# lmcinnes/pynndescent

Measured on AMD Instinct MI355X. Metric: index build: points indexed/sec (recall@10 vs brute force reported alongside), higher is better.
Workload: dtype f32

## Files before the change

### include/pynnd_amd.h

```cpp
#ifndef PYNND_AMD_H
#define PYNND_AMD_H

#include <stdint.h>

#ifdef __cplusplus
extern "C" {
#endif

#define NND_METRIC_SQEUCLIDEAN 0
#define NND_METRIC_ALT_COSINE 1
#define NND_METRIC_ALT_DOT 2
#define NND_METRIC_ALT_INNER_PRODUCT 3
#define NND_METRIC_CORRELATION 4
#define NND_METRIC_ALT_HELLINGER 5
enum { NND_METRIC_PROXY_INNER_PRODUCT = 6 };
enum {
    NND_METRIC_JACCARD = 8,
    NND_METRIC_DICE = 9,
    NND_METRIC_SOKALSNEATH = 10,
    NND_METRIC_MATCHING = 11,
    NND_METRIC_ROGERSTANIMOTO = 12,
    NND_METRIC_SOKALMICHENER = 13,
    NND_METRIC_KULSINSKI = 14,
    NND_METRIC_RUSSELLRAO = 15,
// ... 12 lines not shown
    int32_t n_trees;
    int32_t leaf_size;
    int32_t max_depth;
    int32_t max_candidates;
    int32_t n_iters;
    float delta;
    int64_t rng_state[3];
    int64_t tree_rng[3];
    int32_t device;
    int32_t join_blocks;
    int32_t flags;
    int32_t reserved[5];
} nnd_params;

#define NND_FLAG_NO_GRAPH 1
#define NND_FLAG_NO_PREP 2
#define NND_FLAG_TEST_SELECT_WAVE 4
#define NND_FLAG_TEST_SMALL_REGIONS 8
#define NND_FLAG_TEST_ROUTE_PLAIN 16
#define NND_FLAG_TEST_FOREST_BY_TREE 32
#define NND_FLAG_TEST_FAIL 64
#define NND_FLAG_TEST_VANISH 128
#define NND_FLAG_TEST_SAMPLE_ATOMIC 256
#define NND_FLAG_TEST_FOREST_FALLBACK_TOPS 512
#define NND_FLAG_TEST_FOREST_FALLBACK_SHARE 1024
#define NND_TEST_FALLBACK_AT(flags) ((((flags) & 512) ? 1 : 0) + (((flags) & 1024) ? 2 : 0))
#define NND_FLAG_TEST_SAMPLE_NOMEM 2048
#define NND_FLAG_TEST_SELECT_HALF 4096
#define NND_FLAG_TEST_GATHER_INLINE 8192
#define NND_FLAG_TEST_JOIN_UNSTAGED 16384

#define NND_FLAG_TEST_EXACT_F64 32768
#define NND_FLAG_TEST_RANDOM_INIT_ROWWISE 65536

typedef struct nnd_stats {
    int64_t n_iters_run;
    int64_t n_leaves;
    int64_t tree_levels;
    int64_t leaf_pairs;
    int64_t leaf_rows;
    int64_t join_pairs[64];
    int64_t join_rows[64];
    int64_t join_active[64];
    int64_t proposals[64];
    int64_t updates[64];
    float ms_prep, ms_forest, ms_leaf_init, ms_random_init, ms_descent, ms_finalize;
    float ms_sample[64], ms_join[64], ms_merge[64];
    int64_t join_mfma[64];
    int64_t leaf_mfma;
    int64_t n_cells;
    int64_t join_substeps[64];
} nnd_stats;

int32_t nnd_abi_version(void);
const char *nnd_last_global_error(void);
const char *nnd_last_error(nnd_handle_t h);

int32_t nnd_create(nnd_handle_t *out, const nnd_params *params);
int32_t nnd_destroy(nnd_handle_t h);
int32_t nnd_release_pending(void);

int32_t nnd_host_copy(void *dst, const void *src, int64_t bytes);
int32_t nnd_host_sqrt_f32(float *dst, const float *src, int64_t count);
void *nnd_host_alloc(int64_t bytes);
int32_t nnd_host_free(void *p);

// ... 254 lines not shown
```

### pynndescent_amd/_capi.py

```python
import ctypes as C
import os

import numpy as np

_HERE = os.path.dirname(os.path.abspath(__file__))
LIB_PATH = os.environ.get("PYNND_AMD_LIB", os.path.join(_HERE, "libpynnd_amd.so"))

NND_METRIC_SQEUCLIDEAN = 0
NND_METRIC_ALT_COSINE = 1
NND_METRIC_ALT_DOT = 2
NND_METRIC_ALT_INNER_PRODUCT = 3
NND_METRIC_CORRELATION = 4
NND_METRIC_ALT_HELLINGER = 5
NND_METRIC_PROXY_INNER_PRODUCT = 6
METRIC_CODES = {"euclidean": NND_METRIC_SQEUCLIDEAN, "l2": NND_METRIC_SQEUCLIDEAN, "sqeuclidean": NND_METRIC_SQEUCLIDEAN,
                "cosine": NND_METRIC_ALT_COSINE, "dot": NND_METRIC_ALT_DOT, "inner_product": NND_METRIC_ALT_INNER_PRODUCT,
                "correlation": NND_METRIC_CORRELATION, "hellinger": NND_METRIC_ALT_HELLINGER,
                "proxy_inner_product": NND_METRIC_PROXY_INNER_PRODUCT}
(NND_METRIC_JACCARD, NND_METRIC_DICE, NND_METRIC_SOKALSNEATH, NND_METRIC_MATCHING, NND_METRIC_ROGERSTANIMOTO,
 NND_METRIC_SOKALMICHENER, NND_METRIC_KULSINSKI, NND_METRIC_RUSSELLRAO, NND_METRIC_YULE) = range(8, 17)
BOOLEAN_METRIC_CODES = {"jaccard": NND_METRIC_JACCARD, "dice": NND_METRIC_DICE, "sokalsneath": NND_METRIC_SOKALSNEATH,
                        "matching": NND_METRIC_MATCHING, "rogerstanimoto": NND_METRIC_ROGERSTANIMOTO,
                        "sokalmichener": NND_METRIC_SOKALMICHENER, "kulsinski": NND_METRIC_KULSINSKI,
                        "russellrao": NND_METRIC_RUSSELLRAO, "yule": NND_METRIC_YULE}


def metric_code(name):
    return METRIC_CODES[name] if name in METRIC_CODES else BOOLEAN_METRIC_CODES[name]
NND_DTYPE_FLOAT32, NND_DTYPE_FLOAT16, NND_DTYPE_BFLOAT16, NND_DTYPE_FLOAT64 = 0, 1, 2, 3
NND_FILTER_MASK, NND_FILTER_IDS = 0, 1
NND_QUERY_FORMS = {"float": 0, "proxy": 1, "rerank": 2}
NND_CORRECT_COPY, NND_CORRECT_SQRT, NND_CORRECT_ALT_COSINE, NND_CORRECT_ALT_INNER_PRODUCT, NND_CORRECT_ALT_HELLINGER = 0, 1, 2, 3, 4
NND_LINEAR_DIAGONAL, NND_LINEAR_DENSE = 0, 1
NND_FLAG_NO_GRAPH = 1
NND_FLAG_NO_PREP = 2
NND_FLAG_TEST_SELECT_WAVE = 4
NND_FLAG_TEST_SMALL_REGIONS = 8
NND_FLAG_TEST_ROUTE_PLAIN = 16
NND_FLAG_TEST_FOREST_BY_TREE = 32
NND_FLAG_TEST_FAIL = 64
NND_FLAG_TEST_VANISH = 128
NND_FLAG_TEST_FOREST_FALLBACK_TOPS = 512
NND_FLAG_TEST_FOREST_FALLBACK_SHARE = 1024
NND_FLAG_TEST_GATHER_INLINE = 8192
NND_FLAG_TEST_JOIN_UNSTAGED = 16384
NND_FLAG_TEST_SELECT_HALF = 4096
NND_FLAG_TEST_SAMPLE_NOMEM = 2048
NND_FLAG_TEST_EXACT_F64 = 32768
NND_FLAG_TEST_RANDOM_INIT_ROWWISE = 65536
NND_FLAG_TEST_SAMPLE_ATOMIC = 256


class NNDParams(C.Structure):
    _fields_ = [
        ("n", C.c_int64),
        ("dim", C.c_int32),
        ("metric", C.c_int32),
        ("n_neighbors", C.c_int32),
        ("n_trees", C.c_int32),
        ("leaf_size", C.c_int32),
        ("max_depth", C.c_int32),
        ("max_candidates", C.c_int32),
        ("n_iters", C.c_int32),
        ("delta", C.c_float),
        ("rng_state", C.c_int64 * 3),
        ("tree_rng", C.c_int64 * 3),
        ("device", C.c_int32),
        ("join_blocks", C.c_int32),
        ("flags", C.c_int32),
        ("reserved", C.c_int32 * 5),
    ]


class NNDSearchGraphStats(C.Structure):
    _fields_ = [("forward_nnz", C.c_int64), ("reverse_nnz", C.c_int64), ("union_nnz", C.c_int64), ("final_nnz", C.c_int64),
                ("min_distance", C.c_float), ("max_degree_out", C.c_int32), ("ms_device", C.c_float), ("reserved", C.c_int32 * 3)]


class NNDStats(C.Structure):
    _fields_ = [
        ("n_iters_run", C.c_int64),
        ("n_leaves", C.c_int64),
# ... 972 lines not shown
```

### pynndescent_amd/csrc/rpforest.hip

```cpp
#include <atomic>
#include <chrono>

#include "common.h"
#include "metric.h"
#include "state.h"

#define RP_EPS 1e-8f

static constexpr int SCAN_ITEMS = 8;
static constexpr int SCAN_BLOCK = 256;
static constexpr int SCAN_TILE = SCAN_ITEMS * SCAN_BLOCK;

__global__ void k_forest_init(int32_t *__restrict__ perm, int32_t *__restrict__ pos_seg, uint8_t *__restrict__ leaf_flag,
                              int32_t *__restrict__ inv, int64_t n, int64_t P, int splittable) {
    int64_t g = (int64_t)blockIdx.x * blockDim.x + threadIdx.x;
    if (g >= P) return;
    int64_t t = g / n;
    int64_t i = g - t * n;
    perm[g] = (int32_t)i;
    inv[g] = splittable ? (int32_t)t : -1;
    pos_seg[g] = splittable ? (int32_t)t : -1;
    leaf_flag[g] = (!splittable && i == 0) ? 1 : 0;
}
__global__ void k_forest_init_segs(int32_t *__restrict__ seg_start, int32_t *__restrict__ seg_len, int n_trees,
// ... 482 lines not shown
        return;
    }
    int a = seg_start[s];
    int nl = nleft[s];
    int right;
    int64_t dest;
    if (nl < 0) {
        nl = -nl - 1;
        int off = (int)(g - a);
        right = off & 1;
        dest = right ? (int64_t)a + nl + (off >> 1) : (int64_t)a + (off >> 1);
    } else {
        int L = scan[g] - scan[a];
        right = side[g];
        dest = right ? (int64_t)a + nl + ((int)(g - a) - L) : (int64_t)a + L;
    }
    int32_t p = perm[g];
    perm_out[dest] = p;
    pos_seg_out[dest] = seg_child[2 * s + right];
    if (inv) inv[(g / n) * n + p] = seg_child[2 * s + right];
}

#ifndef NND_FIN_MAX
#define NND_FIN_MAX 2048
#endif
static constexpr int FIN_MAX = NND_FIN_MAX;
#ifndef NND_BIG_MAX
#define NND_BIG_MAX 8192
#endif
static constexpr int BIG_MAX = NND_BIG_MAX;
static constexpr int FIN_STACK = 40;
static constexpr int FIN_SMALL = 512;
static constexpr int FIN_WS = 40;

__device__ __forceinline__ void rp_top2_push(uint64_t &a, uint64_t &b, uint64_t k) {
    if (k < a) {
        b = a;
        a = k;
    } else if (k < b) {
        b = k;
    }
}
__device__ __forceinline__ uint64_t rp_shfl_xor_u64(uint64_t v, int o) {
    const uint32_t lo = (uint32_t)__shfl_xor((int)(uint32_t)v, o, 64), hi = (uint32_t)__shfl_xor((int)(uint32_t)(v >> 32), o, 64);
    return ((uint64_t)hi << 32) | lo;
}

struct rp_record {
    float *hf;
    uint16_t *hh;
    int32_t *child;
    int32_t *leaf_depth;
    int hs, node_top, down_base, lvl_end;
    int *counter, *overflow;
    int min_len, max_len;
};
struct rp_tree_map {
    int tree_bias = 0;
    const int32_t *tree_begin = nullptr;
    int n_tree_begin = 0;
};
__device__ __forceinline__ uint32_t rp_tree_of(const rp_tree_map &tm, int64_t a, int64_t n) {
    if (!tm.tree_begin) return (uint32_t)(a / n) + (uint32_t)tm.tree_bias;
    int t = 0;
    for (int q = 1; q < tm.n_tree_begin; q++) t = a >= tm.tree_begin[q] ? q : t;
    return (uint32_t)t;
}

template <bool BIG, int NTHR, int CAP, bool RECORD = false>
__global__ __launch_bounds__(NTHR, NTHR == 64 ? 5 : 1) void k_finish_subtrees(const float *__restrict__ xp, const uint16_t *__restrict__ xh,
                                                         const float2 *__restrict__ nr, int metric, int dp, int64_t n,
                                                         int32_t *__restrict__ perm,
                                                         const int32_t *__restrict__ seg_start,
                                                         const int32_t *__restrict__ seg_len,
                                                         const int32_t *__restrict__ seg_depth, int depth0, int n_segs,
                                                         int angular, uint32_t seed, int max_depth, int leaf_size,
                                                         uint8_t *__restrict__ leaf_flag, int32_t *__restrict__ tmp_g,
                                                         uint8_t *__restrict__ side_g, int fin_max,
                                                         int32_t *__restrict__ fin_start, int32_t *__restrict__ fin_len,
                                                         int32_t *__restrict__ fin_depth, long long *__restrict__ fin_count,
                                                         rp_tree_map tm, const float *__restrict__ scal, rp_record rec = rp_record{}) {
    extern __shared__ __attribute__((aligned(16))) unsigned char fsm[];
    const int s = blockIdx.x;
    if (s >= n_segs) return;
    const int a = seg_start[s], len = seg_len[s];
    if (len <= 0) return;
    if (RECORD && (len < rec.min_len || len > rec.max_len)) return;
    constexpr int NLDS = BIG ? 0 : CAP;
    constexpr int NW = NTHR / 64;
    int32_t *ids = BIG ? perm + a : (int32_t *)fsm;
    int32_t *tmp = BIG ? tmp_g + a : (int32_t *)fsm + NLDS;
    uint8_t *sd = BIG ? side_g + a : (uint8_t *)((int32_t *)fsm + 2 * NLDS);
    float *h = (float *)(fsm + (size_t)NLDS * 9);
    uint16_t *hb = (uint16_t *)(h + dp + 4);
    int32_t *stk = (int32_t *)(hb + dp);
    int32_t *wsum = stk + FIN_STACK * 4;
    uint64_t *wkeys = (uint64_t *)(wsum + 8);
    const int tid = threadIdx.x, lane = nnd_lane(), w = tid >> 6;
    const uint32_t seedt = seed ^ (rp_tree_of(tm, a, n) * 0x9E3779B9u);
    const float hsc = scal[0], hinv = 1.0f / hsc, inv_s2 = scal[1];
    float cellA = 0.0f, cellB = 0.0f;
    if (!BIG) {
        for (int i = tid; i < len; i += NTHR) {
            const int32_t id = perm[a + i];
            ids[i] = id;
            const float2 nrv = nr[id];
            const float xnm = nnd_metric_unit(metric) ? nrv.x : sqrtf(nrv.x);
            cellA = fmaxf(cellA, nrv.y + RP_ACC * xnm);
            cellB = fmaxf(cellB, xnm + nrv.y);
        }
        cellA = nnd_wave_max_f32_u(cellA);
        cellB = nnd_wave_max_f32_u(cellB);
        if (NW > 1) {
            if (lane == 0) {
                ((float *)wsum)[w] = cellA;
                ((float *)wsum)[8 + w] = cellB;
            }
            __syncthreads();
#pragma unroll
            for (int q = 0; q < NW; q++) {
                cellA = fmaxf(cellA, ((float *)wsum)[q]);
                cellB = fmaxf(cellB, ((float *)wsum)[8 + q]);
            }
            __syncthreads();
        }
    }
    if (tid == 0) {
        stk[0] = 0; stk[1] = len; stk[2] = seg_depth ? seg_depth[s] : depth0;
        stk[3] = RECORD ? rec.node_top - s : 0;
        wsum[7] = 1;
    }
    __syncthreads();
    while (true) {
        const int sp = wsum[7];
        if (sp == 0) break;
        const int ss = stk[(sp - 1) * 4], l = stk[(sp - 1) * 4 + 1], dep = stk[(sp - 1) * 4 + 2], me = stk[(sp - 1) * 4 + 3];
        __syncthreads();
        if (tid == 0) wsum[7] = sp - 1;
        if (!(l > leaf_size && (max_depth - dep) > 0)) {
            if (tid == 0 && l > 0) leaf_flag[a + ss] = 1;
            if (!RECORD && l > 1) {
                for (int i = tid; i < l; i += NTHR) {
                    const int32_t id = ids[ss + i];
                    int r = 0;
                    for (int j = 0; j < l; j++) r += ids[ss + j] < id ? 1 : 0;
                    tmp[r] = id;
                }
                __syncthreads();
                for (int i = tid; i < l; i += NTHR) ids[ss + i] = tmp[i];
            }
            __syncthreads();
            continue;
        }
        if (BIG && l <= fin_max) {
            if (tid == 0) {
                const int idx = (int)atomicAdd((unsigned long long *)fin_count, 1ull);
                fin_start[idx] = a + ss;
                fin_len[idx] = l;
                fin_depth[idx] = dep;
            }
            __syncthreads();
            continue;
        }
        uint64_t k1 = ~0ull, k2 = ~0ull;
        for (int i = tid; i < l; i += NTHR) {
            const uint32_t id = (uint32_t)ids[ss + i];
            rp_top2_push(k1, k2, ((uint64_t)nnd_hash3(seedt, id, (uint32_t)(2 * dep)) << 32) | id);
        }
        {
            const uint64_t g1 = nnd_wave_min_u64_u(k1);
            const uint64_t g2 = nnd_wave_min_u64_u(k1 == g1 ? k2 : k1);
            k1 = g1;
            k2 = g2;
        }
        if (lane == 0) {
            wkeys[2 * w] = k1;
            wkeys[2 * w + 1] = k2;
        }
        __syncthreads();
        k1 = k2 = ~0ull;
#pragma unroll
        for (int q = 0; q < 2 * NW; q++) rp_top2_push(k1, k2, wkeys[q]);
        const int64_t idl = (int64_t)(uint32_t)k1, idr = (int64_t)(uint32_t)k2;
        const float *xl = xp + idl * dp;
        const float *xr = xp + idr * dp;
        float part = 0.0f, psq = 0.0f;
        for (int j = tid; j < dp; j += NTHR) {
            const float lv = xl[j], rv = xr[j];
            const float v = lv - rv;
            h[j] = v;
            part += angular ? v * v : v * (lv + rv);
            psq += v * v;
        }
        part = nnd_wave_sum_f32_u(part);
        psq = nnd_wave_sum_f32_u(psq);
        if (lane == 0) {
            ((float *)wsum)[w] = part;
        }
        __syncthreads();
        float tot = 0.0f;
#pragma unroll
        for (int q = 0; q < NW; q++) tot += ((float *)wsum)[q];
        __syncthreads();
        if (lane == 0) ((float *)wsum)[w] = psq;
        __syncthreads();
        float totsq = 0.0f;
#pragma unroll
        for (int q = 0; q < NW; q++) totsq += ((float *)wsum)[q];
        __syncthreads();
        if (angular) {
            const float nh = sqrtf(tot);
            const float inv = nh < RP_EPS ? 1.0f : 1.0f / nh;
            for (int j = tid; j < dp; j += NTHR) h[j] *= inv;
            if (tid == 0) { h[dp] = 0.0f; h[dp + 1] = nh * inv; }
        } else if (tid == 0) {
            h[dp] = -0.5f * tot;
            h[dp + 1] = sqrtf(totsq);
        }
        __syncthreads();
        float pres = 0.0f;
        for (int j = tid; j < dp; j += NTHR) {
            const float v = h[j];
            const uint16_t b = nnd_f32_to_h16(v, hsc);
            hb[j] = b;
            const float e = v - nnd_h16_to_f32(b, hinv);
            pres += e * e;
        }
        pres = nnd_wave_sum_f32_u(pres);
        if (lane == 0) ((float *)wsum)[w] = pres;
        __syncthreads();
        float rhv = 0.0f;
#pragma unroll
        for (int q = 0; q < NW; q++) rhv += ((float *)wsum)[q];
        rhv = sqrtf(rhv) * 1.000001f;
        if (RECORD) {
            float *rh = rec.hf + (int64_t)me * rec.hs;
            uint16_t *rb = rec.hh + (int64_t)me * dp;
            for (int j = tid; j < dp; j += NTHR) {
                rh[j] = h[j];
                rb[j] = hb[j];
            }
            if (tid == 0) {
                rh[dp] = h[dp];
                rh[dp + 1] = h[dp + 1];
                rh[dp + 2] = rhv;
            }
        }
        const int sub = tid & 3, grp = tid >> 2;
        const int nch = dp >> 3;
        const float off = h[dp], hnorm = h[dp + 1];
        const uint4 *h8 = (const uint4 *)hb;
        constexpr int GQ = NTHR / 4;
        for (int i0 = 0; i0 < l; i0 += 2 * GQ) {
            int64_t pt[2];
            float acc[2], xn[2], rxv[2];
#pragma unroll
            for (int u = 0; u < 2; u++) {
                const int i = i0 + u * GQ + grp;
                pt[u] = ids[ss + (i < l ? i : 0)];
                acc[u] = 0.0f;
            }
            if (BIG) {
#pragma unroll
                for (int u = 0; u < 2; u++) {
                    const float2 nrv = nr[pt[u]];
                    xn[u] = nrv.x;
                    rxv[u] = nrv.y;
                }
            }
            for (int c = sub; c < nch; c += 16) {
                uint4 q[2][4], p[4];
#pragma unroll
                for (int u = 0; u < 2; u++)
#pragma unroll
                    for (int j = 0; j < 4; j++) q[u][j] = ((const uint4 *)(xh + pt[u] * dp))[c + 4 * j < nch ? c + 4 * j : c];
#pragma unroll
                for (int j = 0; j < 4; j++) p[j] = h8[c + 4 * j < nch ? c + 4 * j : c];
#pragma unroll
                for (int u = 0; u < 2; u++)
#pragma unroll
                    for (int j = 0; j < 4; j++)
                        if (c + 4 * j < nch) acc[u] = rp_dot8(q[u][j], p[j], acc[u]);
            }
#pragma unroll
            for (int u = 0; u < 2; u++) {
                const int i = i0 + u * GQ + grp;
                if (i >= l) continue;
                const float m = rp_quad_sum(acc[u]) * inv_s2 + off;
                const float band = BIG ? rp_band(nnd_metric_unit(metric) ? xn[u] : sqrtf(xn[u]), rxv[u], hnorm, rhv) : hnorm * cellA + rhv * cellB + RP_EPS;
                const uint8_t side = rp_side(m, band, xp + pt[u] * dp, h, off, dp, sub, seedt, (uint32_t)pt[u], dep);
                if (sub == 0) sd[i] = side;
            }
        }
        __syncthreads();
        const int per = (l + NTHR - 1) / NTHR;
        const int b0 = tid * per < l ? tid * per : l, b1 = b0 + per < l ? b0 + per : l;
        int cntl, incl, nl, woff;
        for (int attempt = 0;; attempt++) {
            cntl = 0;
            for (int i = b0; i < b1; i++) cntl += sd[i] == 0;
            incl = nnd_wave_incl_scan_i32(cntl);
            if (lane == 63) wsum[w] = incl;
            __syncthreads();
            woff = 0;
            for (int i = 0; i < w; i++) woff += wsum[i];
            nl = 0;
#pragma unroll
            for (int q = 0; q < NW; q++) nl += wsum[q];
            if (nl != 0 && nl != l) break;
            __syncthreads();
            for (int i = b0; i < b1; i++) {
                const uint32_t id = (uint32_t)ids[ss + i];
                sd[i] = attempt == 0 ? (uint8_t)(nnd_hash3(seedt ^ 0x5bd1e995u, id, (uint32_t)(2 * dep + 1)) & 1u)
                                     : (uint8_t)((int64_t)id == idl ? 0 : 1);
            }
            __syncthreads();
        }
        int run = woff + incl - cntl;
        for (int i = b0; i < b1; i++) {
            int dest;
            if (sd[i] == 0) dest = run++;
            else dest = nl + (i - run);
            tmp[dest] = ids[ss + i];
        }
        __syncthreads();
        for (int i = tid; i < l; i += NTHR) ids[ss + i] = tmp[i];
        if (tid == 0) {
            int top = wsum[7];
            const bool left_big = nl >= l - nl;
#pragma unroll
            for (int q = 0; q < 2; q++) {
                const bool left = (q == 0) == left_big;
                const int cs = left ? ss : ss + nl, cl = left ? nl : l - nl;
                int cid = 0;
                if (RECORD) {
                    bool split = cl > leaf_size && (max_depth - (dep + 1)) > 0;
                    if (split) {
                        cid = rec.down_base - atomicAdd(rec.counter, 1);
                        if (cid <= rec.lvl_end) {
                            *rec.overflow = 1;
                            split = false;
                        }
                    }
                    if (!split) {
                        rec.child[2 * me + (left ? 0 : 1)] = -2 - (a + cs);
                        leaf_flag[a + cs] = 1;
                        rec.leaf_depth[a + cs] = dep + 1;
                        continue;
                    }
                    rec.child[2 * me + (left ? 0 : 1)] = cid;
                }
                stk[top * 4] = cs; stk[top * 4 + 1] = cl; stk[top * 4 + 2] = dep + 1; stk[top * 4 + 3] = cid;
                top++;
            }
            wsum[7] = top;
        }
        __syncthreads();
    }
    if (!BIG)
        for (int i = tid; i < len; i += NTHR) perm[a + i] = ids[i];
}

__global__ void k_leaf_starts(const uint8_t *__restrict__ leaf_flag, const int32_t *__restrict__ scan, int64_t P,
                              int32_t *__restrict__ leaf_start) {
    int64_t g = (int64_t)blockIdx.x * blockDim.x + threadIdx.x;
    if (g < P && leaf_flag[g]) leaf_start[scan[g]] = (int32_t)g;
}
__global__ void k_leaf_lens(const int32_t *__restrict__ leaf_start, int64_t n_leaves, int64_t n, int64_t P,
                            int32_t *__restrict__ leaf_len, int32_t *__restrict__ max_len) {
    int64_t i = (int64_t)blockIdx.x * blockDim.x + threadIdx.x;
    int len = 0;
    if (i < n_leaves) {
        int64_t a = leaf_start[i];
        int64_t e = i + 1 < n_leaves ? leaf_start[i + 1] : P;
        int64_t tree_end = (a / n + 1) * n;
        if (e > tree_end) e = tree_end;
        len = (int)(e - a);
        leaf_len[i] = len;
    }
#pragma unroll
    for (int o = 32; o > 0; o >>= 1) {
        const int other = __shfl_xor(len, o, 64);
        len = other > len ? other : len;
    }
    if (nnd_lane() == 0 && len > 0) atomicMax(max_len, len);
}
__global__ void k_tree_leaf_begin(const int32_t *__restrict__ scan, int n_trees, int64_t n, const int32_t *__restrict__ tree_begin,
                                  int64_t P, int32_t n_leaves, long long *__restrict__ out) {
    int t = blockIdx.x * blockDim.x + threadIdx.x;
    if (t >= n_trees) return;
    const int64_t g = tree_begin ? tree_begin[t] : (int64_t)t * n;
    out[t] = g < P ? scan[g] : n_leaves;
}
// ... 664 lines not shown
#define FOREST_HIP_CHECK(expr) NND_HIP_CHECK_AS(expr, #expr, FOREST_ERROR)

static forest_rc run_scan(nnd_ctx *ctx, int mode, const int32_t *pos_seg, uint8_t *bytes, int32_t *total_dev, int64_t P, int64_t n,
                          const int32_t *perm = nullptr) {
    int nb = (int)((P + SCAN_TILE - 1) / SCAN_TILE);
    hipLaunchKernelGGL(k_scan_reduce, dim3(nb), dim3(SCAN_BLOCK), 0, ctx->stream, mode, pos_seg, bytes, P, ctx->scan_blk, perm,
                       ctx->side_pt, n);
    hipLaunchKernelGGL(k_scan_apply<true>, dim3(nb), dim3(SCAN_BLOCK), 0, ctx->stream, mode == 2 ? 0 : mode, pos_seg, bytes, P,
                       ctx->scan_blk, ctx->scan_out, total_dev);
    FOREST_HIP_CHECK(hipGetLastError());
    return FOREST_OK;
}

static forest_rc scan_i32_inplace(nnd_ctx *ctx, int32_t *data, int64_t n, int32_t *total_dev) {
    if (n <= SCAN_TILE) {
        hipLaunchKernelGGL(k_scan_blocks, dim3(1), dim3(256), 0, ctx->stream, data, (int)n, total_dev);
    } else {
        const int nb = (int)((n + SCAN_TILE - 1) / SCAN_TILE);
        hipLaunchKernelGGL(k_scan_i32_reduce, dim3(nb), dim3(SCAN_BLOCK), 0, ctx->stream, data, n, ctx->scan_blk);
        hipLaunchKernelGGL(k_scan_blocks, dim3(1), dim3(256), 0, ctx->stream, ctx->scan_blk, nb, total_dev);
        hipLaunchKernelGGL(k_scan_i32_apply, dim3(nb), dim3(SCAN_BLOCK), 0, ctx->stream, data, n, ctx->scan_blk);
    }
    FOREST_HIP_CHECK(hipGetLastError());
    return FOREST_OK;
}

static forest_rc read_scan_total(nnd_ctx *ctx, int32_t *out) {
    FOREST_HIP_CHECK(hipMemcpyAsync(&ctx->h_pin->scan_total, nnd_scan_total(ctx), sizeof(int32_t), hipMemcpyDeviceToHost, ctx->stream));
    FOREST_HIP_CHECK(nnd_sync_spin(ctx));
    *out = ctx->h_pin->scan_total;
    return FOREST_OK;
}

static size_t fin_smem_bytes(int dp, int cap ) {
    const size_t tail = sizeof(float) * (dp + 4) + sizeof(uint16_t) * dp + sizeof(int32_t) * (FIN_STACK * 4 + FIN_WS);
    return (size_t)cap * 9 + tail;
}

struct forest_rows {
    const float *xp;
    const uint16_t *xh;
    const float2 *nr;
    int64_t n;
    int leaf_size;
};
static forest_rows whole_set_rows(const nnd_ctx *ctx) { return {ctx->xp, ctx->xh, ctx->nr2, ctx->n, ctx->p.leaf_size}; }

struct forest_view {
    forest_rows rows;
    int64_t P;
    int fin_max;
    bool record;
    int T = 0;
    rp_tree_map tm;
    int cur = 0, depth = 0;
    int64_t S = 0;
    long long active_pos = 0;
    int64_t node_base = 0;
    bool inv_live = true;
    nnd_level_flag *flag_dev = nullptr;
    std::vector<int64_t> level_base;
    int64_t n_low = 0, high_lo = 0;
};

template <bool BIG, int NTHR, int CAP, bool RECORD = false>
static forest_rc launch_finisher(nnd_ctx *ctx, const forest_rows &r, int32_t *perm, int32_t *other, const nnd_work_list &wl, int depth0,
                                 long long count, const rp_tree_map &tm, const rp_record &rec = rp_record{}) {
    const nnd_work_list fin = nnd_fin_list(ctx);
    hipLaunchKernelGGL((k_finish_subtrees<BIG, NTHR, CAP, RECORD>), dim3((unsigned)count), dim3(NTHR), fin_smem_bytes(ctx->dp, CAP), ctx->stream,
                       r.xp, r.xh, r.nr, ctx->p.metric, ctx->dp, r.n, perm, wl.start, wl.len, wl.depth, depth0, (int)count,
                       nnd_metric_unit(ctx->p.metric), ctx->tree_seed, ctx->p.max_depth, r.leaf_size, ctx->leaf_flag,
                       BIG ? other : (int32_t *)nullptr, BIG ? ctx->side : (uint8_t *)nullptr, FIN_MAX, fin.start, fin.len, fin.depth,
                       ctx->counters + CNT_FIN_COUNT, tm, ctx->mean + ctx->dp, rec);
    FOREST_HIP_CHECK(hipGetLastError());
    return FOREST_OK;
}

static forest_rc read_fin_count(nnd_ctx *ctx, long long *out) {
    FOREST_HIP_CHECK(hipMemcpyAsync(&ctx->h_pin->fin_count, ctx->counters + CNT_FIN_COUNT, sizeof(long long), hipMemcpyDeviceToHost, ctx->stream));
    FOREST_HIP_CHECK(nnd_sync_spin(ctx));
    *out = ctx->h_pin->fin_count;
    return FOREST_OK;
}

static forest_rc launch_finishers(nnd_ctx *ctx, int32_t *perm, int32_t *other, const nnd_work_list &big, int depth0, long long n_big,
                                  long long n_small, const rp_tree_map &tm) {
    const forest_rows rows = whole_set_rows(ctx);
    forest_rc rc;
    if (n_small > 0 && (rc = launch_finisher<false, 64, FIN_SMALL>(ctx, rows, perm, other, nnd_small_list(ctx), 0, n_small, tm))) return rc;
    if (n_big > 0 && (rc = launch_finisher<true, 256, 0>(ctx, rows, perm, other, big, depth0, n_big, tm))) return rc;
    long long nfin = 0;
    if ((rc = read_fin_count(ctx, &nfin))) return rc;
    if (nfin > ctx->max_segs) {
        ctx->set_error("rp-forest: %lld finisher segments exceed the allocation of %lld", nfin, (long long)ctx->max_segs);
        return FOREST_ERROR;
    }
    if (nfin > 0) return launch_finisher<false, 256, FIN_MAX>(ctx, rows, perm, other, nnd_fin_list(ctx), 0, nfin, tm);
    return FOREST_OK;
}

static forest_rc levels_start(nnd_ctx *ctx, forest_view &v) {
    const int64_t n = v.rows.n;
// ... 83 lines not shown
    }
    volatile long long *seqw = &ctx->h_pin->flag.seq;
    const auto t_spin = std::chrono::steady_clock::now();
    unsigned spins = 0;
    while (*seqw != ctx->flag_seq) {
        if ((++spins & 0xFFFFu) == 0 && std::chrono::steady_clock::now() - t_spin > std::chrono::seconds(30)) {
            ctx->set_error("rp-forest: the device did not hand over the segment count of level %d within 30 s", v.depth);
            return FOREST_ERROR;
        }
    }
    std::atomic_thread_fence(std::memory_order_acquire);
    *next = ctx->h_pin->flag.w;
    return FOREST_OK;
}

static forest_rc record_subtrees(nnd_ctx *ctx, forest_view &v) {
    const int64_t node_base = v.node_base;
    v.level_base.push_back(node_base);
    forest_rc rc;
    long long nfin = 0;
    if ((rc = read_fin_count(ctx, &nfin))) return rc;
    if (nfin > ctx->max_segs || node_base + nfin + 1 >= ctx->node_cap) return forest_fallback("the subtrees to record outgrow the node tables");
    v.n_low = node_base;
    v.high_lo = ctx->node_cap;
    if (nfin == 0) return FOREST_OK;
    int *flags = (int *)(ctx->counters + CNT_REC_FLAGS);
    FOREST_HIP_CHECK(hipMemsetAsync(flags, 0, 2 * sizeof(int), ctx->stream));
    rp_record rec{ctx->node_hf, ctx->node_hh, ctx->node_child, ctx->s_leaf_depth, ctx->dp + 4, (int)ctx->node_cap - 1,
                  (int)(ctx->node_cap - 1 - nfin), (int)node_base, flags, flags + 1, 0, FIN_MAX};
    rp_record rs = rec, rl = rec;
    rs.min_len = 0; rs.max_len = FIN_SMALL;
    rl.min_len = FIN_SMALL + 1; rl.max_len = FIN_MAX;
    const nnd_work_list fin = nnd_fin_list(ctx);
    if ((rc = launch_finisher<false, 64, FIN_SMALL, true>(ctx, v.rows, ctx->perm[v.cur], nullptr, fin, 0, nfin, v.tm, rs))) return rc;
    if (v.fin_max > FIN_SMALL && (rc = launch_finisher<false, 256, FIN_MAX, true>(ctx, v.rows, ctx->perm[v.cur], nullptr, fin, 0, nfin, v.tm, rl)))
        return rc;
    FOREST_HIP_CHECK(hipMemcpyAsync(ctx->h_pin->rec_flags, flags, 2 * sizeof(int), hipMemcpyDeviceToHost, ctx->stream));
    FOREST_HIP_CHECK(nnd_sync_spin(ctx));
    if (ctx->h_pin->rec_flags[1]) return forest_fallback("the recording finisher ran out of node slots");
    v.high_lo = ctx->node_cap - nfin - ctx->h_pin->rec_flags[0];
    return FOREST_OK;
}

static forest_rc forest_levels(nnd_ctx *ctx, forest_view &v) {
    forest_rc rc = levels_start(ctx, v);
    if (rc) return rc;
    while (v.S > 0) {
        nnd_level_words next;
        if ((rc = level_launch(ctx, v)) || (rc = level_handover(ctx, v, &next))) return rc;
        v.node_base += v.S;
        v.S = next.segs;
        v.active_pos = next.active_pos;
        v.cur = 1 - v.cur;
        v.depth++;
        if (!v.record && v.S > 0 && (v.active_pos * 2 < 3 * v.rows.n) && next.max_stay <= BIG_MAX) {
            const nnd_work_list stayers{ctx->seg_start[v.cur], ctx->seg_len[v.cur], nullptr};
            return launch_finishers(ctx, ctx->perm[v.cur], ctx->perm[1 - v.cur], stayers, v.depth, v.S, 0, v.tm);
        }
    }
    if (v.record) return record_subtrees(ctx, v);
    return launch_finishers(ctx, ctx->perm[v.cur], ctx->perm[1 - v.cur], nnd_work_list{}, 0, 0, 0, v.tm);
}

static forest_rc device_cus(nnd_ctx *ctx, int *out) {
    static int n_cu_dev[64] = {0};
    int &n_cu = n_cu_dev[ctx->p.device & 63];
    if (n_cu == 0) {
        hipDeviceProp_t prop;
        FOREST_HIP_CHECK(hipGetDeviceProperties(&prop, ctx->p.device));
// ... 512 lines not shown
```

Measured before the change: 54.86 million.

## Process sibling subtree nodes in parallel waves and defer node recording in finisher

The recording subtree finisher for small segments now runs four waves per block, each handling a different node of the same tree level from an LDS work list, instead of one wave walking a serial stack. Node hyperplanes are recorded afterwards: node ids are numbered locally in LDS and reserved with a single atomicAdd per subtree, and the planes are then recomputed and written out. The large-segment recorder also adopts the deferred numbering. This trades recomputing each node's plane and extra LDS for more parallelism and fewer global atomics, with a test flag that keeps the old serial path.

```diff
diff --git a/include/pynnd_amd.h b/include/pynnd_amd.h
--- a/include/pynnd_amd.h
+++ b/include/pynnd_amd.h
@@ -68,6 +68,7 @@
 
 #define NND_FLAG_TEST_EXACT_F64 32768
 #define NND_FLAG_TEST_RANDOM_INIT_ROWWISE 65536
+#define NND_FLAG_TEST_FINISH_SERIAL 131072
 
 typedef struct nnd_stats {
     int64_t n_iters_run;
diff --git a/pynndescent_amd/_capi.py b/pynndescent_amd/_capi.py
--- a/pynndescent_amd/_capi.py
+++ b/pynndescent_amd/_capi.py
@@ -48,6 +48,7 @@
 NND_FLAG_TEST_SAMPLE_NOMEM = 2048
 NND_FLAG_TEST_EXACT_F64 = 32768
 NND_FLAG_TEST_RANDOM_INIT_ROWWISE = 65536
+NND_FLAG_TEST_FINISH_SERIAL = 131072
 NND_FLAG_TEST_SAMPLE_ATOMIC = 256
 
 
diff --git a/pynndescent_amd/csrc/rpforest.hip b/pynndescent_amd/csrc/rpforest.hip
--- a/pynndescent_amd/csrc/rpforest.hip
+++ b/pynndescent_amd/csrc/rpforest.hip
@@ -538,6 +538,9 @@
 static constexpr int FIN_STACK = 40;
 static constexpr int FIN_SMALL = 512;
 static constexpr int FIN_WS = 40;
+__host__ __device__ constexpr size_t fin_node_smem_bytes(int dp) {
+    return sizeof(float) * (dp + 4) + sizeof(uint16_t) * dp + sizeof(int32_t) * (FIN_STACK * 4 + FIN_WS);
+}
 
 __device__ __forceinline__ void rp_top2_push(uint64_t &a, uint64_t &b, uint64_t k) {
     if (k < a) {
@@ -573,8 +576,75 @@
     return (uint32_t)t;
 }
 
-template <bool BIG, int NTHR, int CAP, bool RECORD = false>
-__global__ __launch_bounds__(NTHR, NTHR == 64 ? 5 : 1) void k_finish_subtrees(const float *__restrict__ xp, const uint16_t *__restrict__ xh,
+static constexpr int FIN_SIBLINGS = 4;
+template <bool WAVE>
+__device__ __forceinline__ void rp_node_sync() {
+    if constexpr (WAVE) nnd_wave_lds_sync();
+    else __syncthreads();
+}
+template <int NTHR, bool WAVE>
+__device__ __forceinline__ float rp_node_plane(const float *__restrict__ xl, const float *__restrict__ xr, int dp, int angular, float hsc,
+                                               float hinv, float *h, uint16_t *hb, int32_t *wsum, int tid) {
+    constexpr int NW = NTHR / 64;
+    const int lane = nnd_lane(), w = tid >> 6;
+    float part = 0.0f, psq = 0.0f;
+    for (int j = tid; j < dp; j += NTHR) {
+        const float lv = xl[j], rv = xr[j];
+        const float v = lv - rv;
+        h[j] = v;
+        part += angular ? v * v : v * (lv + rv);
+        psq += v * v;
+    }
+    part = nnd_wave_sum_f32_u(part);
+    psq = nnd_wave_sum_f32_u(psq);
+    if (lane == 0) {
+        ((float *)wsum)[w] = part;
+    }
+    rp_node_sync<WAVE>();
+    float tot = 0.0f;
+#pragma unroll
+    for (int q = 0; q < NW; q++) tot += ((float *)wsum)[q];
+    rp_node_sync<WAVE>();
+    if (lane == 0) ((float *)wsum)[w] = psq;
+    rp_node_sync<WAVE>();
+    float totsq = 0.0f;
+#pragma unroll
+    for (int q = 0; q < NW; q++) totsq += ((float *)wsum)[q];
+    rp_node_sync<WAVE>();
+    if (angular) {
+        const float nh = sqrtf(tot);
+        const float inv = nh < RP_EPS ? 1.0f : 1.0f / nh;
+        for (int j = tid; j < dp; j += NTHR) h[j] *= inv;
+        if (tid == 0) { h[dp] = 0.0f; h[dp + 1] = nh * inv; }
+    } else if (tid == 0) {
+        h[dp] = -0.5f * tot;
+        h[dp + 1] = sqrtf(totsq);
+    }
+    rp_node_sync<WAVE>();
+    float pres = 0.0f;
+    for (int j = tid; j < dp; j += NTHR) {
+        const float v = h[j];
+        const uint16_t b = nnd_f32_to_h16(v, hsc);
+        hb[j] = b;
+        const float e = v - nnd_h16_to_f32(b, hinv);
+        pres += e * e;
+    }
+    pres = nnd_wave_sum_f32_u(pres);
+    if (lane == 0) ((float *)wsum)[w] = pres;
+    rp_node_sync<WAVE>();
+    float rhv = 0.0f;
+#pragma unroll
+    for (int q = 0; q < NW; q++) rhv += ((float *)wsum)[q];
+    return sqrtf(rhv) * 1.000001f;
+}
+template <int NTHR, bool WAVE>
+__device__ __noinline__ float rp_node_plane_twice(const float *__restrict__ xl, const float *__restrict__ xr, int dp, int angular, float hsc,
+                                                  float hinv, float *h, uint16_t *hb, int32_t *wsum, int tid) {
+    return rp_node_plane<NTHR, WAVE>(xl, xr, dp, angular, hsc, hinv, h, hb, wsum, tid);
+}
+
+template <bool BIG, int NTHR, int CAP, bool RECORD = false, int SIB = 1, bool DEFER = (SIB > 1)>
+__global__ __launch_bounds__(NTHR * SIB, NTHR == 64 ? 5 : 1) void k_finish_subtrees(const float *__restrict__ xp, const uint16_t *__restrict__ xh,
                                                          const float2 *__restrict__ nr, int metric, int dp, int64_t n,
                                                          int32_t *__restrict__ perm,
                                                          const int32_t *__restrict__ seg_start,
@@ -592,22 +662,34 @@
     const int a = seg_start[s], len = seg_len[s];
     if (len <= 0) return;
     if (RECORD && (len < rec.min_len || len > rec.max_len)) return;
+    static_assert(SIB == 1 || (NTHR == 64 && !BIG && RECORD), "the node-parallel form: one wave per node, ids in LDS, recording");
+    static_assert(SIB <= 8 && CAP < (1 << 15), "bred holds 8 waves; a list entry packs start and length into 16 bits each");
+    static_assert(!DEFER || (RECORD && !BIG), "deferred recording: the subtree's node table lives in LDS");
+    static_assert(SIB == 1 || DEFER, "the node-parallel form numbers its nodes itself");
+    constexpr bool WSYNC = SIB > 1;
     constexpr int NLDS = BIG ? 0 : CAP;
     constexpr int NW = NTHR / 64;
+    constexpr int BTHR = NTHR * SIB, BW = NW * SIB;
+    const int btid = threadIdx.x, lane = nnd_lane();
+    const int wv = SIB > 1 ? btid >> 6 : 0;
+    const int tid = SIB > 1 ? lane : btid, w = SIB > 1 ? 0 : btid >> 6;
     int32_t *ids = BIG ? perm + a : (int32_t *)fsm;
     int32_t *tmp = BIG ? tmp_g + a : (int32_t *)fsm + NLDS;
     uint8_t *sd = BIG ? side_g + a : (uint8_t *)((int32_t *)fsm + 2 * NLDS);
-    float *h = (float *)(fsm + (size_t)NLDS * 9);
+    float *h = (float *)(fsm + (size_t)NLDS * 9 + (size_t)wv * fin_node_smem_bytes(dp));
     uint16_t *hb = (uint16_t *)(h + dp + 4);
     int32_t *stk = (int32_t *)(hb + dp);
     int32_t *wsum = stk + FIN_STACK * 4;
     uint64_t *wkeys = (uint64_t *)(wsum + 8);
-    const int tid = threadIdx.x, lane = nnd_lane(), w = tid >> 6;
+    int32_t *ntab = (int32_t *)(fsm + (size_t)NLDS * 9 + (size_t)SIB * fin_node_smem_bytes(dp));
+    int32_t *lcnt = ntab + 4 * CAP;
+    float *bred = (float *)(lcnt + 4);
+    int2 *nlist = (int2 *)(bred + 16);
     const uint32_t seedt = seed ^ (rp_tree_of(tm, a, n) * 0x9E3779B9u);
     const float hsc = scal[0], hinv = 1.0f / hsc, inv_s2 = scal[1];
     float cellA = 0.0f, cellB = 0.0f;
     if (!BIG) {
-        for (int i = tid; i < len; i += NTHR) {
+        for (int i = btid; i < len; i += BTHR) {
             const int32_t id = perm[a + i];
             ids[i] = id;
             const float2 nrv = nr[id];
@@ -617,32 +699,67 @@
         }
         cellA = nnd_wave_max_f32_u(cellA);
         cellB = nnd_wave_max_f32_u(cellB);
-        if (NW > 1) {
+        if (BW > 1) {
+            float *red = SIB > 1 ? bred : (float *)wsum;
+            const int bw = btid >> 6;
             if (lane == 0) {
-                ((float *)wsum)[w] = cellA;
-                ((float *)wsum)[8 + w] = cellB;
+                red[bw] = cellA;
+                red[8 + bw] = cellB;
             }
             __syncthreads();
 #pragma unroll
-            for (int q = 0; q < NW; q++) {
-                cellA = fmaxf(cellA, ((float *)wsum)[q]);
-                cellB = fmaxf(cellB, ((float *)wsum)[8 + q]);
+            for (int q = 0; q < BW; q++) {
+                cellA = fmaxf(cellA, red[q]);
+                cellB = fmaxf(cellB, red[8 + q]);
             }
             __syncthreads();
         }
     }
-    if (tid == 0) {
-        stk[0] = 0; stk[1] = len; stk[2] = seg_depth ? seg_depth[s] : depth0;
-        stk[3] = RECORD ? rec.node_top - s : 0;
-        wsum[7] = 1;
+    const int dep0 = seg_depth ? seg_depth[s] : depth0;
+    if (btid == 0) {
+        if (SIB > 1) {
+            nlist[0] = make_int2(len << 16, -1);
+            lcnt[0] = 1; lcnt[1] = 0; lcnt[2] = 0;
+            ntab[0] = -1;
+        } else {
+            stk[0] = 0; stk[1] = len; stk[2] = dep0;
+            stk[3] = RECORD && !DEFER ? rec.node_top - s : 0;
+            wsum[7] = 1;
+            if (DEFER) {
+                wsum[6] = 1;
+                ntab[0] = -1;
+            }
+        }
     }
     __syncthreads();
+    [[maybe_unused]] int lvl = -1, qi = 0, nn = 0, id_base = 0;
     while (true) {
-        const int sp = wsum[7];
-        if (sp == 0) break;
-        const int ss = stk[(sp - 1) * 4], l = stk[(sp - 1) * 4 + 1], dep = stk[(sp - 1) * 4 + 2], me = stk[(sp - 1) * 4 + 3];
-        __syncthreads();
-        if (tid == 0) wsum[7] = sp - 1;
+        int ss, l, dep, me;
+        if constexpr (SIB > 1) {
+            if (qi >= nn) {
+                __syncthreads();
+                lvl++;
+                id_base += nn;
+                nn = lcnt[lvl % 3];
+                if (nn == 0) break;
+                if (btid == 0) lcnt[(lvl + 2) % 3] = 0;
+                qi = wv;
+                continue;
+            }
+            const int2 e = nlist[(lvl & 1) * (CAP / 2) + qi];
+            ss = e.x & 0xffff; l = e.x >> 16; dep = dep0 + lvl;
+            me = id_base + qi;
+            qi += SIB;
+            if (tid == 0 && lvl > 0) ntab[e.y] = me;
+        } else {
+            const int sp = wsum[7];
+            if (sp == 0) break;
+            ss = stk[(sp - 1) * 4]; l = stk[(sp - 1) * 4 + 1]; dep = stk[(sp - 1) * 4 + 2]; me = stk[(sp - 1) * 4 + 3];
+            __syncthreads();
+            if (tid == 0) wsum[7] = sp - 1;
+        }
+        int32_t *const tmpn = SIB > 1 ? tmp + ss : tmp;
+        uint8_t *const sdn = SIB > 1 ? sd + ss : sd;
         if (!(l > leaf_size && (max_depth - dep) > 0)) {
             if (tid == 0 && l > 0) leaf_flag[a + ss] = 1;
             if (!RECORD && l > 1) {
@@ -655,7 +772,7 @@
                 __syncthreads();
                 for (int i = tid; i < l; i += NTHR) ids[ss + i] = tmp[i];
             }
-            __syncthreads();
+            rp_node_sync<WSYNC>();
             continue;
         }
         if (BIG && l <= fin_max) {
@@ -683,73 +800,31 @@
             wkeys[2 * w] = k1;
             wkeys[2 * w + 1] = k2;
         }
-        __syncthreads();
+        rp_node_sync<WSYNC>();
         k1 = k2 = ~0ull;
 #pragma unroll
         for (int q = 0; q < 2 * NW; q++) rp_top2_push(k1, k2, wkeys[q]);
         const int64_t idl = (int64_t)(uint32_t)k1, idr = (int64_t)(uint32_t)k2;
         const float *xl = xp + idl * dp;
         const float *xr = xp + idr * dp;
-        float part = 0.0f, psq = 0.0f;
-        for (int j = tid; j < dp; j += NTHR) {
-            const float lv = xl[j], rv = xr[j];
-            const float v = lv - rv;
-            h[j] = v;
-            part += angular ? v * v : v * (lv + rv);
-            psq += v * v;
-        }
-        part = nnd_wave_sum_f32_u(part);
-        psq = nnd_wave_sum_f32_u(psq);
-        if (lane == 0) {
-            ((float *)wsum)[w] = part;
-        }
-        __syncthreads();
-        float tot = 0.0f;
-#pragma unroll
-        for (int q = 0; q < NW; q++) tot += ((float *)wsum)[q];
-        __syncthreads();
-        if (lane == 0) ((float *)wsum)[w] = psq;
-        __syncthreads();
-        float totsq = 0.0f;
-#pragma unroll
-        for (int q = 0; q < NW; q++) totsq += ((float *)wsum)[q];
-        __syncthreads();
-        if (angular) {
-            const float nh = sqrtf(tot);
-            const float inv = nh < RP_EPS ? 1.0f : 1.0f / nh;
-            for (int j = tid; j < dp; j += NTHR) h[j] *= inv;
-            if (tid == 0) { h[dp] = 0.0f; h[dp + 1] = nh * inv; }
-        } else if (tid == 0) {
-            h[dp] = -0.5f * tot;
-            h[dp + 1] = sqrtf(totsq);
-        }
-        __syncthreads();
-        float pres = 0.0f;
-        for (int j = tid; j < dp; j += NTHR) {
-            const float v = h[j];
-            const uint16_t b = nnd_f32_to_h16(v, hsc);
-            hb[j] = b;
-            const float e = v - nnd_h16_to_f32(b, hinv);
-            pres += e * e;
-        }
-        pres = nnd_wave_sum_f32_u(pres);
-        if (lane == 0) ((float *)wsum)[w] = pres;
-        __syncthreads();
-        float rhv = 0.0f;
-#pragma unroll
-        for (int q = 0; q < NW; q++) rhv += ((float *)wsum)[q];
-        rhv = sqrtf(rhv) * 1.000001f;
-        if (RECORD) {
-            float *rh = rec.hf + (int64_t)me * rec.hs;
-            uint16_t *rb = rec.hh + (int64_t)me * dp;
-            for (int j = tid; j < dp; j += NTHR) {
-                rh[j] = h[j];
-                rb[j] = hb[j];
-            }
-            if (tid == 0) {
-                rh[dp] = h[dp];
-                rh[dp + 1] = h[dp + 1];
-                rh[dp + 2] = rhv;
+        float rhv;
+        if constexpr (DEFER) {
+            if (tid == 0) { ntab[4 * me] = (int32_t)idl; ntab[4 * me + 1] = (int32_t)idr; }
+            rhv = rp_node_plane_twice<NTHR, WSYNC>(xl, xr, dp, angular, hsc, hinv, h, hb, wsum, tid);
+        } else {
+            rhv = rp_node_plane<NTHR, WSYNC>(xl, xr, dp, angular, hsc, hinv, h, hb, wsum, tid);
+            if (RECORD) {
+                float *rh = rec.hf + (int64_t)me * rec.hs;
+                uint16_t *rb = rec.hh + (int64_t)me * dp;
+                for (int j = tid; j < dp; j += NTHR) {
+                    rh[j] = h[j];
+                    rb[j] = hb[j];
+                }
+                if (tid == 0) {
+                    rh[dp] = h[dp];
+                    rh[dp + 1] = h[dp + 1];
+                    rh[dp + 2] = rhv;
+                }
             }
         }
         const int sub = tid & 3, grp = tid >> 2;
@@ -795,44 +870,44 @@
                 const float m = rp_quad_sum(acc[u]) * inv_s2 + off;
                 const float band = BIG ? rp_band(nnd_metric_unit(metric) ? xn[u] : sqrtf(xn[u]), rxv[u], hnorm, rhv) : hnorm * cellA + rhv * cellB + RP_EPS;
                 const uint8_t side = rp_side(m, band, xp + pt[u] * dp, h, off, dp, sub, seedt, (uint32_t)pt[u], dep);
-                if (sub == 0) sd[i] = side;
-            }
-        }
-        __syncthreads();
+                if (sub == 0) sdn[i] = side;
+            }
+        }
+        rp_node_sync<WSYNC>();
         const int per = (l + NTHR - 1) / NTHR;
         const int b0 = tid * per < l ? tid * per : l, b1 = b0 + per < l ? b0 + per : l;
         int cntl, incl, nl, woff;
         for (int attempt = 0;; attempt++) {
             cntl = 0;
-            for (int i = b0; i < b1; i++) cntl += sd[i] == 0;
+            for (int i = b0; i < b1; i++) cntl += sdn[i] == 0;
             incl = nnd_wave_incl_scan_i32(cntl);
             if (lane == 63) wsum[w] = incl;
-            __syncthreads();
+            rp_node_sync<WSYNC>();
             woff = 0;
             for (int i = 0; i < w; i++) woff += wsum[i];
             nl = 0;
 #pragma unroll
             for (int q = 0; q < NW; q++) nl += wsum[q];
             if (nl != 0 && nl != l) break;
-            __syncthreads();
+            rp_node_sync<WSYNC>();
             for (int i = b0; i < b1; i++) {
                 const uint32_t id = (uint32_t)ids[ss + i];
-                sd[i] = attempt == 0 ? (uint8_t)(nnd_hash3(seedt ^ 0x5bd1e995u, id, (uint32_t)(2 * dep + 1)) & 1u)
+                sdn[i] = attempt == 0 ? (uint8_t)(nnd_hash3(seedt ^ 0x5bd1e995u, id, (uint32_t)(2 * dep + 1)) & 1u)
                                      : (uint8_t)((int64_t)id == idl ? 0 : 1);
             }
-            __syncthreads();
+            rp_node_sync<WSYNC>();
         }
         int run = woff + incl - cntl;
         for (int i = b0; i < b1; i++) {
             int dest;
-            if (sd[i] == 0) dest = run++;
+            if (sdn[i] == 0) dest = run++;
             else dest = nl + (i - run);
-            tmp[dest] = ids[ss + i];
-        }
-        __syncthreads();
-        for (int i = tid; i < l; i += NTHR) ids[ss + i] = tmp[i];
+            tmpn[dest] = ids[ss + i];
+        }
+        rp_node_sync<WSYNC>();
+        for (int i = tid; i < l; i += NTHR) ids[ss + i] = tmpn[i];
         if (tid == 0) {
-            int top = wsum[7];
+            int top = SIB > 1 ? 0 : wsum[7];
             const bool left_big = nl >= l - nl;
 #pragma unroll
             for (int q = 0; q < 2; q++) {
@@ -841,7 +916,8 @@
                 int cid = 0;
                 if (RECORD) {
                     bool split = cl > leaf_size && (max_depth - (dep + 1)) > 0;
-                    if (split) {
+                    if (split && DEFER && SIB == 1) cid = wsum[6]++;
+                    if (split && !DEFER) {
                         cid = rec.down_base - atomicAdd(rec.counter, 1);
                         if (cid <= rec.lvl_end) {
                             *rec.overflow = 1;
@@ -849,22 +925,61 @@
                         }
                     }
                     if (!split) {
-                        rec.child[2 * me + (left ? 0 : 1)] = -2 - (a + cs);
+                        if (DEFER) ntab[4 * me + 2 + (left ? 0 : 1)] = -2 - (a + cs);
+                        else rec.child[2 * me + (left ? 0 : 1)] = -2 - (a + cs);
                         leaf_flag[a + cs] = 1;
                         rec.leaf_depth[a + cs] = dep + 1;
                         continue;
                     }
-                    rec.child[2 * me + (left ? 0 : 1)] = cid;
+                    if (!DEFER) rec.child[2 * me + (left ? 0 : 1)] = cid;
+                    else if (SIB == 1) ntab[4 * me + 2 + (left ? 0 : 1)] = cid;
+                }
+                if (SIB > 1) {
+                    const int at = atomicAdd(&lcnt[(lvl + 1) % 3], 1);
+                    nlist[((lvl + 1) & 1) * (CAP / 2) + at] = make_int2(cs | (cl << 16), 4 * me + 2 + (left ? 0 : 1));
+                    continue;
                 }
                 stk[top * 4] = cs; stk[top * 4 + 1] = cl; stk[top * 4 + 2] = dep + 1; stk[top * 4 + 3] = cid;
                 top++;
             }
-            wsum[7] = top;
-        }
+            if (SIB == 1) wsum[7] = top;
+        }
+        rp_node_sync<WSYNC>();
+    }
+    if constexpr (DEFER) {
+        const int numbered = SIB > 1 ? id_base : wsum[6];
+        const int total = (numbered == 1 && ntab[0] < 0) ? 0 : numbered;
+        if (btid == 0 && total > 1) lcnt[3] = atomicAdd(rec.counter, total - 1);
         __syncthreads();
+        const int first = lcnt[3];
+        for (int i = wv; i < total; i += SIB) {
+            const int nid = i == 0 ? rec.node_top - s : rec.down_base - (first + i - 1);
+            if (nid <= rec.lvl_end) {
+                if (tid == 0) *rec.overflow = 1;
+                continue;
+            }
+            const float rhv = rp_node_plane_twice<NTHR, WSYNC>(xp + (int64_t)ntab[4 * i] * dp, xp + (int64_t)ntab[4 * i + 1] * dp, dp, angular, hsc,
+                                                               hinv, h, hb, wsum, tid);
+            float *rh = rec.hf + (int64_t)nid * rec.hs;
+            uint16_t *rb = rec.hh + (int64_t)nid * dp;
+            for (int j = tid; j < dp; j += NTHR) {
+                rh[j] = h[j];
+                rb[j] = hb[j];
+            }
+            if (tid == 0) {
+                rh[dp] = h[dp];
+                rh[dp + 1] = h[dp + 1];
+                rh[dp + 2] = rhv;
+            }
+            if (tid < 2) {
+                const int c = ntab[4 * i + 2 + tid];
+                rec.child[2 * nid + tid] = c <= -2 ? c : rec.down_base - (first + c - 1);
+            }
+            rp_node_sync<WSYNC>();
+        }
     }
     if (!BIG)
-        for (int i = tid; i < len; i += NTHR) perm[a + i] = ids[i];
+        for (int i = btid; i < len; i += BTHR) perm[a + i] = ids[i];
 }
 
 __global__ void k_leaf_starts(const uint8_t *__restrict__ leaf_flag, const int32_t *__restrict__ scan, int64_t P,
@@ -1595,9 +1710,11 @@
     return FOREST_OK;
 }
 
-static size_t fin_smem_bytes(int dp, int cap ) {
-    const size_t tail = sizeof(float) * (dp + 4) + sizeof(uint16_t) * dp + sizeof(int32_t) * (FIN_STACK * 4 + FIN_WS);
-    return (size_t)cap * 9 + tail;
+static size_t fin_smem_bytes(int dp, int cap , int sib = 1 , bool defer = false) {
+    size_t extra = 0;
+    if (defer) extra += sizeof(int32_t) * 4 * cap + sizeof(int32_t) * 4 + sizeof(float) * 16;
+    if (sib > 1) extra += sizeof(int2) * cap;
+    return (size_t)cap * 9 + (size_t)sib * fin_node_smem_bytes(dp) + extra;
 }
 
 struct forest_rows {
@@ -1626,11 +1743,11 @@
     int64_t n_low = 0, high_lo = 0;
 };
 
-template <bool BIG, int NTHR, int CAP, bool RECORD = false>
+template <bool BIG, int NTHR, int CAP, bool RECORD = false, int SIB = 1, bool DEFER = (SIB > 1)>
 static forest_rc launch_finisher(nnd_ctx *ctx, const forest_rows &r, int32_t *perm, int32_t *other, const nnd_work_list &wl, int depth0,
                                  long long count, const rp_tree_map &tm, const rp_record &rec = rp_record{}) {
     const nnd_work_list fin = nnd_fin_list(ctx);
-    hipLaunchKernelGGL((k_finish_subtrees<BIG, NTHR, CAP, RECORD>), dim3((unsigned)count), dim3(NTHR), fin_smem_bytes(ctx->dp, CAP), ctx->stream,
+    hipLaunchKernelGGL((k_finish_subtrees<BIG, NTHR, CAP, RECORD, SIB, DEFER>), dim3((unsigned)count), dim3(NTHR * SIB), fin_smem_bytes(ctx->dp, CAP, SIB, DEFER), ctx->stream,
                        r.xp, r.xh, r.nr, ctx->p.metric, ctx->dp, r.n, perm, wl.start, wl.len, wl.depth, depth0, (int)count,
                        nnd_metric_unit(ctx->p.metric), ctx->tree_seed, ctx->p.max_depth, r.leaf_size, ctx->leaf_flag,
                        BIG ? other : (int32_t *)nullptr, BIG ? ctx->side : (uint8_t *)nullptr, FIN_MAX, fin.start, fin.len, fin.depth,
@@ -1780,9 +1897,15 @@
     rs.min_len = 0; rs.max_len = FIN_SMALL;
     rl.min_len = FIN_SMALL + 1; rl.max_len = FIN_MAX;
     const nnd_work_list fin = nnd_fin_list(ctx);
-    if ((rc = launch_finisher<false, 64, FIN_SMALL, true>(ctx, v.rows, ctx->perm[v.cur], nullptr, fin, 0, nfin, v.tm, rs))) return rc;
-    if (v.fin_max > FIN_SMALL && (rc = launch_finisher<false, 256, FIN_MAX, true>(ctx, v.rows, ctx->perm[v.cur], nullptr, fin, 0, nfin, v.tm, rl)))
-        return rc;
+    const bool serial = ctx->p.flags & NND_FLAG_TEST_FINISH_SERIAL;
+    if (serial) rc = launch_finisher<false, 64, FIN_SMALL, true>(ctx, v.rows, ctx->perm[v.cur], nullptr, fin, 0, nfin, v.tm, rs);
+    else rc = launch_finisher<false, 64, FIN_SMALL, true, FIN_SIBLINGS>(ctx, v.rows, ctx->perm[v.cur], nullptr, fin, 0, nfin, v.tm, rs);
+    if (rc) return rc;
+    if (v.fin_max > FIN_SMALL) {
+        if (serial) rc = launch_finisher<false, 256, FIN_MAX, true>(ctx, v.rows, ctx->perm[v.cur], nullptr, fin, 0, nfin, v.tm, rl);
+        else rc = launch_finisher<false, 256, FIN_MAX, true, 1, true>(ctx, v.rows, ctx->perm[v.cur], nullptr, fin, 0, nfin, v.tm, rl);
+        if (rc) return rc;
+    }
     FOREST_HIP_CHECK(hipMemcpyAsync(ctx->h_pin->rec_flags, flags, 2 * sizeof(int), hipMemcpyDeviceToHost, ctx->stream));
     FOREST_HIP_CHECK(nnd_sync_spin(ctx));
     if (ctx->h_pin->rec_flags[1]) return forest_fallback("the recording finisher ran out of node slots");
```

Result: faster. 55.49 million, median of 6 (+1.2%).
